# nv-dvl/nerfmatch

Measured on AMD Instinct MI355X. Metric: rays*samples/sec, higher is better.
Workload: dtype fp16x3 (fp16 MFMA on hi/lo-split fp32 operands, three products per fp32 product, fp32 accumulate; fp32 everywhere else)

## Files before the change

### nerfmatch_amd/csrc/nerf_bf16_common.h

```cpp
#pragma once
#include "bf16x3.h"
#include <string.h>

namespace nmbf {

constexpr int TILE = 128;
constexpr int SLOT_BYTES = 16384;
constexpr int SLOT_FLOATS = SLOT_BYTES / 4;
constexpr int NRING = 4;
constexpr int WS_WORKGROUPS = 512;
constexpr int XS = 6;
constexpr int HS = 16;
constexpr int VS = 3;
constexpr int NSLOT_NORGB = XS + 4 * HS + (XS + HS) + 2 * HS;
constexpr int NSLOT_FULL = NSLOT_NORGB + (HS + VS);

constexpr int OFF_BIAS = 0, OFF_BVIEWS = 2304, OFF_WALPHA = 2432, OFF_WRGB = 2688, OFF_MISC = 3072;
constexpr int OFF_SCALE = 3088, OFF_DESCALE = 3104, OFF_INSCALE = 3112, SMALL = 3120;
constexpr int NRANGE = 10;
constexpr int SMALL_PAD = 4096;
constexpr int NSLOT_PAD = 4;
constexpr size_t BLOB_BYTES = (size_t)SMALL_PAD * 4 + (size_t)(NSLOT_FULL + NSLOT_PAD) * SLOT_BYTES;
constexpr int NSLOT_FULL_PAIRED = NSLOT_NORGB + HS / 2 + 2;
constexpr size_t BLOB_BYTES_FP16 = (size_t)SMALL_PAD * 4 + (size_t)(NSLOT_FULL + 8) * (SLOT_BYTES / 2);
constexpr int NSLOT_BWD = 8 + 8 + 16 * 9;
constexpr size_t BLOB_BYTES_BWD = (size_t)SMALL_PAD * 4 + (size_t)(NSLOT_BWD + NSLOT_PAD) * SLOT_BYTES;

constexpr int LDS_SMALL = 0;
constexpr int LDS_RING = SMALL_PAD;
constexpr int LDS_IPE = LDS_RING + NRING * SLOT_FLOATS;
constexpr int LDS_SCR = LDS_IPE + 4 * XS * 2 * 64 * 4;
constexpr int LDS_FEAT = LDS_SCR + TILE * 12 + 32;
constexpr int LDS_EX = LDS_FEAT + 4 * 256;
constexpr int LDS_LEFT = LDS_EX + 4 * 48;
constexpr int LDS_RNG = LDS_LEFT + 2 * TILE;
constexpr int LDS_TOTAL = LDS_RNG + NRANGE * 256;

struct NerfArgs {
  const char* blob;
  const float* rays;
  const float* t;
  const float* app_row;
  float* weights;
  float* feat;
  float* pts;
  float* rgb;
  float* depth;
  float* acc;
  float* raw;
  float* sfeat;
  float* ws;
  int R, S, tap, white_bg, flags, ntiles;
  int Sa;
  int left;
  int ntiles_full;
  const int* tail_viol;
  float var_scale;
  int* status;
};

#ifndef NM_TRACE
#define NM_TRACE 0
#endif

__device__ __forceinline__ int launder(int v) {
  asm volatile("" : "+v"(v));
  return v;
}
__device__ __forceinline__ int launder_s(int v) {
  asm volatile("" : "+s"(v));
  return v;
}

#if NM_TRACE
#define TRACE(i)                                                                                               \
  do {                                                                                                         \
    if (a.raw && threadIdx.x == 0) reinterpret_cast<unsigned long long*>(a.raw)[bid * 32 + (i)] = __builtin_amdgcn_s_memtime(); \
  } while (0)
#else
#define TRACE(i) do { } while (0)
#endif

__device__ __forceinline__ float acc_read(float av) {
  asm volatile("" : "+v"(av));
  return av;
}

template <class T>
__device__ __forceinline__ void pin(T& v) {
  asm volatile("" : "+v"(v));
}
__device__ __forceinline__ float sin32(float x) {
  const float q = __builtin_rintf(x * 0.318309886183790671537767526745028724f);
  float d = __builtin_fmaf(q, -3.140625f, x);
  d = __builtin_fmaf(q, -0.0009670257568359375f, d);
  d = __builtin_fmaf(q, -6.2771141529083251953e-07f, d);
  d = __builtin_fmaf(q, -1.2154201256553420762e-10f, d);
  const float s = d * d;
  d = ((int)q & 1) ? -d : d;
  float u = 2.6083159809786593541503e-06f;
  u = __builtin_fmaf(u, s, -0.0001981069071916863322258f);
  u = __builtin_fmaf(u, s, 0.00833307858556509017944336f);
  u = __builtin_fmaf(u, s, -0.166666597127914428710938f);
  return __builtin_fmaf(s, u * d, d);
}


}
```

### nerfmatch_amd/csrc/nerf_fwd_bf16.hip

```cpp
#include "nerf_split_chain.h"

namespace {
using namespace nmbf;

template <int PART>
__device__ __forceinline__ void tap_prefetch(Ctx& cx) {
  if constexpr (PART == 0) __builtin_amdgcn_s_barrier();
  const char* src = reinterpret_cast<const char*>(cx.tapw);
#pragma unroll
  for (int q = (PART == 0 ? 0 : 4); q < (PART == 0 ? 4 : 7); ++q) {
    const char* sp = src + q * 4096;
    const float* dp = q < 4 ? cx.tap_ring + q * 1024 : cx.tap_ipe + (q - 4) * 1024;
    const unsigned lds = (unsigned)__builtin_amdgcn_readfirstlane((int)(unsigned)(size_t)(const __attribute__((address_space(3))) float*)dp);
    unsigned m0_saved;
    asm volatile("s_mov_b32 %0, m0\n\ts_mov_b32 m0, %1\n\tglobal_load_lds_dwordx4 %2, off\n\tglobal_load_lds_dwordx4 %2, off offset:1024\n\t"
                 "global_load_lds_dwordx4 %2, off offset:2048\n\tglobal_load_lds_dwordx4 %2, off offset:3072\n\ts_mov_b32 m0, %0"
                 : "=&s"(m0_saved) : "s"(lds), "v"(sp) : "memory");
  }
}

__device__ __forceinline__ void dpp_pairs8(float (&o)[8], const float (&x)[8], const float (&y)[8], bool eight) {
  if (eight)
    asm("s_nop 1\n"
        "v_add_f32_dpp %0, %8, %8 row_mirror row_mask:0xf bank_mask:0x3\n\tv_add_f32_dpp %1, %9, %9 row_mirror row_mask:0xf bank_mask:0x3\n\t"
// ... 20 lines not shown
        : "=&v"(o[0]), "=&v"(o[1]), "=&v"(o[2]), "=&v"(o[3]), "=&v"(o[4]), "=&v"(o[5]), "=&v"(o[6]), "=&v"(o[7])
        : "v"(x[0]), "v"(x[1]), "v"(x[2]), "v"(x[3]), "v"(x[4]), "v"(x[5]), "v"(x[6]), "v"(x[7]),
          "v"(y[0]), "v"(y[1]), "v"(y[2]), "v"(y[3]), "v"(y[4]), "v"(y[5]), "v"(y[6]), "v"(y[7]));
}
template <int XOR>
__device__ __forceinline__ void quad_add8(float (&v)[8]) {
  if (XOR == 1)
    asm("s_nop 1\n"
        "v_add_f32_dpp %0, %0, %0 quad_perm:[1,0,3,2] row_mask:0xf bank_mask:0xf\n\tv_add_f32_dpp %1, %1, %1 quad_perm:[1,0,3,2] row_mask:0xf bank_mask:0xf\n\t"
        "v_add_f32_dpp %2, %2, %2 quad_perm:[1,0,3,2] row_mask:0xf bank_mask:0xf\n\tv_add_f32_dpp %3, %3, %3 quad_perm:[1,0,3,2] row_mask:0xf bank_mask:0xf\n\t"
        "v_add_f32_dpp %4, %4, %4 quad_perm:[1,0,3,2] row_mask:0xf bank_mask:0xf\n\tv_add_f32_dpp %5, %5, %5 quad_perm:[1,0,3,2] row_mask:0xf bank_mask:0xf\n\t"
        "v_add_f32_dpp %6, %6, %6 quad_perm:[1,0,3,2] row_mask:0xf bank_mask:0xf\n\tv_add_f32_dpp %7, %7, %7 quad_perm:[1,0,3,2] row_mask:0xf bank_mask:0xf"
        : "+v"(v[0]), "+v"(v[1]), "+v"(v[2]), "+v"(v[3]), "+v"(v[4]), "+v"(v[5]), "+v"(v[6]), "+v"(v[7]));
  else
    asm("s_nop 1\n"
        "v_add_f32_dpp %0, %0, %0 quad_perm:[2,3,0,1] row_mask:0xf bank_mask:0xf\n\tv_add_f32_dpp %1, %1, %1 quad_perm:[2,3,0,1] row_mask:0xf bank_mask:0xf\n\t"
        "v_add_f32_dpp %2, %2, %2 quad_perm:[2,3,0,1] row_mask:0xf bank_mask:0xf\n\tv_add_f32_dpp %3, %3, %3 quad_perm:[2,3,0,1] row_mask:0xf bank_mask:0xf\n\t"
        "v_add_f32_dpp %4, %4, %4 quad_perm:[2,3,0,1] row_mask:0xf bank_mask:0xf\n\tv_add_f32_dpp %5, %5, %5 quad_perm:[2,3,0,1] row_mask:0xf bank_mask:0xf\n\t"
        "v_add_f32_dpp %6, %6, %6 quad_perm:[2,3,0,1] row_mask:0xf bank_mask:0xf\n\tv_add_f32_dpp %7, %7, %7 quad_perm:[2,3,0,1] row_mask:0xf bank_mask:0xf"
        : "+v"(v[0]), "+v"(v[1]), "+v"(v[2]), "+v"(v[3]), "+v"(v[4]), "+v"(v[5]), "+v"(v[6]), "+v"(v[7]));
}
__device__ __forceinline__ float reduce_scatter_step16(float x, float y) {
  const auto r = __builtin_amdgcn_permlane16_swap(__float_as_uint(x), __float_as_uint(y), false, false);
  return __uint_as_float(r[0]) + __uint_as_float(r[1]);
}
__device__ __forceinline__ f32x4 reduce_scatter_16pairs(const float (&s1)[64], int lane) {
  float s2[32];
#pragma unroll
  for (int b = 0; b < 4; ++b) {
    float o[8], x[8], y[8];
#pragma unroll
    for (int i = 0; i < 8; ++i) { x[i] = s1[8 * b + i]; y[i] = s1[32 + 8 * b + i]; }
    dpp_pairs8(o, x, y, true);
#pragma unroll
    for (int i = 0; i < 8; ++i) s2[8 * b + i] = o[i];
  }
  float s3[16];
#pragma unroll
  for (int b = 0; b < 2; ++b) {
    float o[8], x[8], y[8];
#pragma unroll
    for (int i = 0; i < 8; ++i) { x[i] = s2[8 * b + i]; y[i] = s2[16 + 8 * b + i]; }
    dpp_pairs8(o, x, y, false);
#pragma unroll
    for (int i = 0; i < 8; ++i) s3[8 * b + i] = o[i];
  }
  float lo8[8], hi8[8];
#pragma unroll
  for (int i = 0; i < 8; ++i) { lo8[i] = s3[i]; hi8[i] = s3[8 + i]; }
  quad_add8<2>(lo8); quad_add8<2>(hi8);
  float s4[8];
#pragma unroll
  for (int i = 0; i < 8; ++i) s4[i] = (lane & 2) ? hi8[i] : lo8[i];
  float t8[8] = {s4[0], s4[1], s4[2], s4[3], s4[4], s4[5], s4[6], s4[7]};
  quad_add8<1>(t8);
  return (lane & 1) ? f32x4{t8[4], t8[5], t8[6], t8[7]} : f32x4{t8[0], t8[1], t8[2], t8[3]};
}
__device__ __forceinline__ f32x4 reduce_scatter_32rows(float (&v)[128], int lane) {
  float s1[64];
#pragma unroll
  for (int i = 0; i < 64; ++i) s1[i] = reduce_scatter_step16(v[i], v[64 + i]);
  return reduce_scatter_16pairs(s1, lane);
}

#define NM_MLP_DONE_WAIT() __builtin_amdgcn_s_waitcnt(0x0070)
#define NM_EPI_BARRIER() asm volatile("s_waitcnt lgkmcnt(0)\n\ts_barrier" ::: "memory")
template <int P>
__device__ __forceinline__ void nerf_fwd_body(const NerfArgs& a) {
  __shared__ __attribute__((aligned(16))) float sm[LDS_TOTAL];
  float* const sm_small = sm + LDS_SMALL;
  float* const ring = sm + LDS_RING;
  float* const sm_ipe = sm + LDS_IPE;
  float* const sm_sigma = sm + LDS_SCR;
  float* const sm_rgb = sm_sigma + TILE;
  float* const sm_t0 = sm_rgb + 3 * TILE;
  float* const sm_t1 = sm_t0 + TILE;
  float* const sm_mean = sm_t1 + TILE;
  float* const sm_dn = sm_mean + 3 * TILE;
  float* const sm_w = sm_dn + TILE;
  float* const sm_misc = sm_w + TILE;
  float* const sm_part = sm_misc + 32;
  float* const sm_feat = sm + LDS_FEAT;
  float* const sm_ex = sm + LDS_EX;
  int* const sm_lray = reinterpret_cast<int*>(sm + LDS_LEFT);
  float* const sm_lT = sm + LDS_LEFT + TILE;
  unsigned* const sm_rng = reinterpret_cast<unsigned*>(sm + LDS_RNG);

  const int tid = threadIdx.x, lane = tid & 63, wave = tid >> 6, s = lane & 31, hi = lane >> 5;
  const bool tail_ok = a.left && !(a.tail_viol && *a.tail_viol != 0);
  const int S = a.S, R = a.R;
  const int Sa = tail_ok ? a.Sa : S;
  const int left = tail_ok ? 1 : 0;
  const int ntiles = tail_ok ? a.ntiles : a.ntiles_full;
  const int SP = Sa < TILE ? Sa : TILE;
  const int nr = TILE / SP;
  const int nchunks = (Sa + TILE - 1) / TILE;
  const bool need_rgb = !(a.flags & NM_NERF_SKIP_RGB);
  const bool feat_max = (a.flags & NM_NERF_FEAT_MAX) != 0;
  const bool need_tap = (a.feat != nullptr) || (a.sfeat != nullptr);
  const int tap = (a.tap < 0 || a.tap > 7) ? 7 : a.tap;
  const int nslots = need_rgb ? NSLOT_FULL : NSLOT_NORGB;
  const char* const blob_slots = a.blob + (size_t)SMALL_PAD * 4;

  for (int i = tid; i < SMALL / 4; i += 256) reinterpret_cast<f32x4*>(sm_small)[i] = reinterpret_cast<const f32x4*>(a.blob)[i];
  if constexpr (P == 2) {
#pragma unroll
    for (int k = 0; k < NRANGE; ++k) sm_rng[k * 256 + tid] = 0u;
  }

  int nleft = 0;
  int bid = blockIdx.x;
#pragma unroll 1
  for (;;) {
  bool lo_pass = false;
  if (left && (nleft > TILE - 4 || (bid >= ntiles && nleft > 0))) lo_pass = true;
  else if (bid >= ntiles) break;
  const int nent = lo_pass ? nleft : 0;
  TRACE(0);
  if (need_rgb && !lo_pass && tid < nr * 48) {
    const int r2 = tid / 48, f = tid % 48;
    const int ray2 = bid * nr + r2;
    const float* rq = a.rays + (size_t)(ray2 < R ? ray2 : R - 1) * 12 + 8;
    float v = 0.f;
    if (f < 24) {
      const int k = (f % 12) / 3;
      const float xe = rq[f % 3] * (float)(1 << k);
      v = nm_sinf(f < 12 ? xe : xe + 1.57079637050628662109375f);
    } else if (f < 27) {
      v = rq[f - 24];
    } else if (f < 43) {
      v = a.app_row ? a.app_row[f - 27] : 0.f;
    }
    if constexpr (P == 2) {
      v *= reinterpret_cast<const float*>(a.blob)[OFF_INSCALE + (f < 27 ? 1 : 2)];
      __hip_atomic_fetch_max(sm_rng + 9 * 256 + tid, __float_as_uint(fabsf(v)), __ATOMIC_RELAXED, __HIP_MEMORY_SCOPE_WORKGROUP);
    }
    sm_ex[tid] = v;
  }
  __syncthreads();
  TRACE(1);

  const int js = wave * 32 + s;
  const int rl = js / SP;
  const int ray = lo_pass ? (js < nent ? sm_lray[js] : R) : bid * nr + rl;
  const int rc = lo_pass ? sm_lray[js < nent ? js : 0] : (ray < R ? ray : R - 1);
  const float* rp = a.rays + (size_t)rc * 12;
  const float o0 = rp[0], o1 = rp[1], o2 = rp[2], d0 = rp[3], d1 = rp[4], d2 = rp[5], radius = rp[11];
  const float dsq0 = d0 * d0, dsq1 = d1 * d1, dsq2 = d2 * d2;
  const float dmag = fmaxf(1e-10f, (dsq0 + dsq1) + dsq2);
  const float dnorm = sqrtf((dsq0 + dsq1) + dsq2);
  const float nul0 = 1.0f - dsq0 / dmag, nul1 = 1.0f - dsq1 / dmag, nul2 = 1.0f - dsq2 / dmag;

  float red_acc = 0.f;
  float carryT = 1.f;
  float best_w = -1.f;
  float feat_run = 0.f;

  const int nch = lo_pass ? 1 : nchunks;
  for (int chunk = 0; chunk < nch; ++chunk) {
    const int sidx = lo_pass ? Sa : chunk * TILE + (js % SP);
    const float t0 = a.t[(size_t)rc * (S + 1) + sidx];
    const float t1 = a.t[(size_t)rc * (S + 1) + sidx + 1];
    const float mu = (t0 + t1) / 2.0f, hw = (t1 - t0) / 2.0f;
    const float mu2 = mu * mu, hw2 = hw * hw, hw4 = hw2 * hw2;
    const float denom = fmaxf(1.1920928955078125e-07f, 3.0f * mu2 + hw2);
    const float t_mean = mu + (2.0f * mu * hw2) / denom;
    const float t_var = hw2 / 3.0f - (float)(4.0 / 15.0) * ((hw4 * (12.0f * mu2 - hw2)) / (denom * denom));
    const float r_var = (radius * radius) * ((mu2 / 4.0f + (float)(5.0 / 12.0) * hw2) - (float)(4.0 / 15.0) * hw4 / denom);
    float mean[3] = {d0 * t_mean + o0, d1 * t_mean + o1, d2 * t_mean + o2};
    float var[3] = {t_var * dsq0 + r_var * nul0, t_var * dsq1 + r_var * nul1, t_var * dsq2 + r_var * nul2};
    if (a.var_scale > 0.f) {
      var[0] *= a.var_scale; var[1] *= a.var_scale; var[2] *= a.var_scale;
    }
    if (hi == 0) {
      sm_t0[js] = t0; sm_t1[js] = t1;
      sm_mean[js] = mean[0]; sm_mean[TILE + js] = mean[1]; sm_mean[2 * TILE + js] = mean[2];
      sm_dn[js] = dnorm;
    }

#pragma unroll
    for (int g0 = 0; g0 < ring_ahead<P>(); ++g0) dma_slot<P>(blob_slots, g0, ring, wave, lane);

    {
      float* dst = sm_ipe + wave * (XS * 2 * 64 * 4) + lane * 4;
      const float ipe_scale = sm_small[OFF_INSCALE];
      const float phl = hi ? 1.57079637050628662109375f : 0.f;
#pragma unroll
      for (int m = 0; m < XS; ++m) {
        float v8[8];
#pragma unroll
        for (int i = 0; i < 8; ++i) {
          const int idx = 8 * m + i;
          const bool live = idx < 45;
          const int ax = (live ? idx : 0) % 3, sb = (live ? idx : 0) / 3;
          const float mu = mean[ax], vr = var[ax];
          const float sc = (float)(1 << sb);
          const float xe = mu * sc;
          float v = __builtin_amdgcn_exp2f((-0.5f * (vr * (sc * sc))) * 1.44269504088896340736f) * sin32(xe + phl);
          if constexpr (P == 2) v *= ipe_scale;
          v8[i] = live ? v : 0.f;
        }
        if constexpr (is_split<P>()) {
          bf16x8 h8, l8;
          split8_p<P>(v8, h8, l8);
          *reinterpret_cast<u32x4*>(dst + (m * 2 + 0) * 256) = __builtin_bit_cast(u32x4, h8);
          *reinterpret_cast<u32x4*>(dst + (m * 2 + 1) * 256) = __builtin_bit_cast(u32x4, l8);
        } else {
          *reinterpret_cast<u32x4*>(dst + m * 256) = __builtin_bit_cast(u32x4, pack8_f16(v8));
        }
      }
    }

    TRACE(2);
    Ctx cx;
    cx.blob_slots = blob_slots; cx.ring = ring; cx.sm_small = sm_small;
    cx.tapw = reinterpret_cast<f32x4*>(a.ws) + ((size_t)blockIdx.x * 4 + wave) * 32 * 64 + lane;
    cx.nslots = nslots; cx.wave = wave; cx.lane = lane; cx.hi = hi; cx.tap = need_tap ? tap : -1; cx.g = 0; cx.sig_part = 0.f;
    cx.vmax = 0.f; cx.rng = sm_rng + tid; cx.sc = 1.f;
    const bool early = need_rgb && !lo_pass && tap == 7 && a.feat && !a.sfeat;
    cx.tap_pref = need_tap && !lo_pass && !early; cx.rgb = need_rgb;
// ... 54 lines not shown
          if (a.raw && !NM_TRACE) {
            f32x4 rv = {sm_rgb[tid2], sm_rgb[TILE + tid2], sm_rgb[2 * TILE + tid2], sm_sigma[tid2]};
            *reinterpret_cast<f32x4*>(a.raw + ((size_t)ray2 * S + s2) * 4) = rv;
          }
        }
        float pq[8] = {wgt, wgt * sm_rgb[tid2], wgt * sm_rgb[TILE + tid2], wgt * sm_rgb[2 * TILE + tid2],
                       wgt * (0.5f * (sm_t0[tid2] + sm_t1[tid2])), wgt * sm_mean[tid2], wgt * sm_mean[TILE + tid2],
                       wgt * sm_mean[2 * TILE + tid2]};
        nm_half_sum_dpp8(pq);
        if ((tid2 & 31) == 16) {
          *reinterpret_cast<f32x4*>(sm_part + (tid2 >> 5) * 8) = f32x4{pq[0], pq[1], pq[2], pq[3]};
          *reinterpret_cast<f32x4*>(sm_part + (tid2 >> 5) * 8 + 4) = f32x4{pq[4], pq[5], pq[6], pq[7]};
        }
      }
    };
    auto pick_best = [&]() __attribute__((always_inline)) {
      const int tid2 = launder(threadIdx.x);
      if (tid2 < 8 * nr) {
        const int q = tid2 & 7, r2 = tid2 >> 3;
        const float* wv = sm_w + r2 * SP;
        float bw = wv[0];
        int bi = 0;
        for (int k = 1; k < SP; ++k)
          if (wv[k] > bw) { bw = wv[k]; bi = k; }
        const bool better = bw > best_w;
        if (better) best_w = bw;
        if (q == 0) sm_misc[8 + r2] = better ? __int_as_float(r2 * SP + bi) : __int_as_float(-1);
        if (q >= 5 && better) red_acc = sm_mean[(q - 5) * TILE + r2 * SP + bi];
      }
    };
    auto tap7_early = [&](Ctx& c) __attribute__((always_inline)) {
      const int t2 = launder(threadIdx.x), jl = (t2 >> 6) * 32 + (t2 & 31), hl = (t2 >> 5) & 1;
      const float sigma_raw = (c.sig_part + nm_shfl_xor32(c.sig_part)) + sm_small[OFF_MISC];
      if (hl == 0) sm_sigma[jl] = sigma_raw;
      NM_EPI_BARRIER();
      composite_weights();
      NM_EPI_BARRIER();
      if (feat_max) {
        pick_best();
        NM_EPI_BARRIER();
      }
      const float desc = sm_small[OFF_DESCALE + 7];
      const float wj = sm_w[jl] * desc;
      const int best = feat_max ? __float_as_int(sm_misc[8 + jl / SP]) : -2;
      const float mult = feat_max ? (jl == best ? desc : 0.f) : wj;
      const float* bl = sm_small + OFF_BIAS + 7 * 256 + 4 * hl;
      const float s7 = sm_small[OFF_SCALE + 7];
      float s1[64];
#pragma unroll
      for (int cq = 0; cq < HS; ++cq) {
        const f32x4 b0 = *reinterpret_cast<const f32x4*>(bl + (cq >> 2) * 32 + 8 * (cq & 3));
        const f32x4 b1 = *reinterpret_cast<const f32x4*>(bl + (4 + (cq >> 2)) * 32 + 8 * (cq & 3));
#pragma unroll
        for (int e = 0; e < 4; ++e) {
          const float x = mult * __builtin_fmaxf(__builtin_fmaf(c.hv[4 * cq + e], s7, b0[e]), 0.f);
          const float y = mult * __builtin_fmaxf(__builtin_fmaf(c.hv[64 + 4 * cq + e], s7, b1[e]), 0.f);
          s1[4 * cq + e] = reduce_scatter_step16(x, y);
        }
      }
      const f32x4 sum4 = reduce_scatter_16pairs(s1, jl);
      const int r = jl & 31;
      float* prow = sm_feat + (jl >> 5) * 256 + 4 * hl;
      *reinterpret_cast<f32x4*>(prow + (r >> 2) * 32 + 16 * ((r >> 1) & 1) + 8 * (r & 1)) = sum4;
    };
    const Tap7InRegisters<decltype(tap7_early)> tap7{early, tap7_early};
    f32x16 acc[8];
    ipe_steps<P, true>(acc, cx, ipe_src);
    finish_layer<P>(acc, 0, cx);
    TRACE(3);
#pragma unroll 1
    for (int l = 1; l < 8; ++l) {
      layer_pass<P>(acc, l, cx, ipe_src, tap7);
      TRACE(3 + l);
    }
    float c_r = 0.f, c_g = 0.f, c_b = 0.f;
    if (!need_rgb) {
      if (cx.tap == 7) dump_tap(7, cx);
      NM_MLP_DONE_WAIT();
      if (cx.tap_pref) tap_prefetch<0>(cx);
      alpha_head(cx);
      if (cx.tap_pref) tap_prefetch<1>(cx);
    } else {
      const int hh = launder(lane) >> 5;
      const float* exr = sm_ex + launder(rl) * 48 + 8 * hh;
      f32x16 av[4];
      views_hidden<P>(av, cx);
      fold_range<P>(cx, 7);
      bf16x8 exh[VS], exl[VS];
#pragma unroll
      for (int e = 0; e < VS; ++e) {
        float v8[8];
        if (!lo_pass) {
          const f32x4 e0 = *reinterpret_cast<const f32x4*>(exr + 16 * e), e1 = *reinterpret_cast<const f32x4*>(exr + 16 * e + 4);
          v8[0] = e0[0]; v8[1] = e0[1]; v8[2] = e0[2]; v8[3] = e0[3]; v8[4] = e1[0]; v8[5] = e1[1]; v8[6] = e1[2]; v8[7] = e1[3];
        } else {
          const float* rq = a.rays + (size_t)launder(rc) * 12 + 8;
          const float vd0 = rq[0], vd1 = rq[1], vd2 = rq[2];
#pragma unroll
          for (int i = 0; i < 8; ++i) {
            const int f = 16 * e + 8 * hh + i;
            const int ax = f % 3;
            const float dax = ax == 0 ? vd0 : ax == 1 ? vd1 : vd2;
            float v = 0.f;
            if (f < 24) {
              const float xe = dax * (float)(1 << ((f % 12) / 3));
              v = nm_sinf(f < 12 ? xe : xe + 1.57079637050628662109375f);
            } else if (f < 27) {
              v = dax;
            } else if (f < 43) {
              v = a.app_row ? a.app_row[f - 27] : 0.f;
            }
            if constexpr (P == 2) v *= sm_small[OFF_INSCALE + (f < 27 ? 1 : 2)];
            v8[i] = v;
          }
        }
        if constexpr (is_split<P>()) split8_p<P>(v8, exh[e], exl[e]);
        else exh[e] = exl[e] = pack8_f16(v8);
      }
      views_extras<P>(av, cx, exh, exl);
      TRACE(11);
      NM_MLP_DONE_WAIT();
      if (cx.tap_pref) tap_prefetch<0>(cx);
      const float* bv = sm_small + OFF_BVIEWS + 4 * hh;
      const float* wr = sm_small + OFF_WRGB + 4 * hh;
      float pr = 0.f, pg = 0.f, pb = 0.f;
#pragma unroll
      for (int ob = 0; ob < 4; ++ob) {
#pragma unroll
        for (int q = 0; q < 4; ++q) {
          const f32x4 b4 = *reinterpret_cast<const f32x4*>(bv + ob * 32 + 8 * q);
          const f32x4 wr4 = *reinterpret_cast<const f32x4*>(wr + ob * 32 + 8 * q);
          const f32x4 wg4 = *reinterpret_cast<const f32x4*>(wr + 128 + ob * 32 + 8 * q);
          const f32x4 wb4 = *reinterpret_cast<const f32x4*>(wr + 256 + ob * 32 + 8 * q);
#pragma unroll
          for (int e = 0; e < 4; ++e) {
            const float hv = __builtin_fmaxf(acc_read(av[ob][4 * q + e]) + b4[e], 0.f);
            pr = NM_FMA(hv, wr4[e], pr);
            pg = NM_FMA(hv, wg4[e], pg);
            pb = NM_FMA(hv, wb4[e], pb);
          }
        }
      }
      pr = (pr + nm_shfl_xor32(pr)) + sm_small[OFF_MISC + 1];
      pg = (pg + nm_shfl_xor32(pg)) + sm_small[OFF_MISC + 2];
      pb = (pb + nm_shfl_xor32(pb)) + sm_small[OFF_MISC + 3];
      c_r = 1.0f / (1.0f + expf(-pr));
      c_g = 1.0f / (1.0f + expf(-pg));
      c_b = 1.0f / (1.0f + expf(-pb));
      if (cx.tap_pref) tap_prefetch<1>(cx);
    }
    const float sigma_raw = (cx.sig_part + nm_shfl_xor32(cx.sig_part)) + sm_small[OFF_MISC];
    TRACE(12);
    {
      const int jsw = launder(js);
      if ((launder(lane) >> 5) == 0) {
        sm_sigma[jsw] = sigma_raw;
        sm_rgb[jsw] = c_r; sm_rgb[TILE + jsw] = c_g; sm_rgb[2 * TILE + jsw] = c_b;
      }
    }
    NM_EPI_BARRIER();
    TRACE(13);
    const int tid2 = launder(threadIdx.x), lane2 = tid2 & 63, wave2 = tid2 >> 6;

    if (lo_pass) {
      if (tid2 < nent) {
        const int ray2 = sm_lray[tid2];
        const float sg = fmaxf(sm_sigma[tid2], 0.f);
        const float delta = (sm_t1[tid2] - sm_t0[tid2]) * sm_dn[tid2];
        const float wgt = (1.0f - expf(-sg * delta)) * sm_lT[tid2];
        sm_w[tid2] = wgt;
        a.weights[(size_t)ray2 * S + Sa] = wgt;
        if (a.acc) atomicAdd(a.acc + ray2, wgt);
        if (a.rgb && need_rgb) {
#pragma unroll
          for (int c = 0; c < 3; ++c) atomicAdd(a.rgb + (size_t)ray2 * 3 + c, a.white_bg ? wgt * sm_rgb[c * TILE + tid2] - wgt : wgt * sm_rgb[c * TILE + tid2]);
        }
        if (a.depth) atomicAdd(a.depth + ray2, wgt * (0.5f * (sm_t0[tid2] + sm_t1[tid2])));
        if (a.pts) {
#pragma unroll
          for (int c = 0; c < 3; ++c) atomicAdd(a.pts + (size_t)ray2 * 3 + c, wgt * sm_mean[c * TILE + tid2]);
        }
      }
      __syncthreads();
      if (need_tap) {
        const int jl = launder(js), hl = launder(lane) >> 5;
        const f32x4* tw = reinterpret_cast<const f32x4*>(a.ws) + ((size_t)blockIdx.x * 4 + wave2) * 32 * 64 + lane2;
        if (jl < nent) {
          const int ray2 = sm_lray[jl];
          const float desc = sm_small[OFF_DESCALE + tap];
          const float wj = sm_w[jl] * desc;
#pragma unroll 4
          for (int ks = 0; ks < HS; ++ks) {
            const f32x4 ta = tw[(2 * ks) * 64], tb = tw[(2 * ks + 1) * 64];
            const int n0 = (ks >> 1) * 32 + 16 * (ks & 1) + 4 * hl;
            if (a.sfeat) {
              float* dsf = a.sfeat + ((size_t)ray2 * S + Sa) * 256 + n0;
              *reinterpret_cast<f32x4*>(dsf) = ta * desc;
              *reinterpret_cast<f32x4*>(dsf + 8) = tb * desc;
            }
            if (a.feat) {
              float* df = a.feat + (size_t)ray2 * 256 + n0;
#pragma unroll
              for (int e = 0; e < 4; ++e) {
                atomicAdd(df + e, wj * ta[e]);
                atomicAdd(df + 8 + e, wj * tb[e]);
              }
            }
          }
        }
      }
      __syncthreads();
      break;
    }

    if (!early) composite_weights();
    composite_sums();
    NM_EPI_BARRIER();

    if (tid2 < 8 * nr) {
// ... 173 lines not shown
```

### nerfmatch_amd/csrc/nerf_pack_bf16.hip

```cpp
#include "nerf_bf16_common.h"
#include <stdlib.h>

namespace {
using namespace nmbf;

inline uint16_t bf16_rne(float f) {
  uint32_t u;
  memcpy(&u, &f, 4);
  if ((u & 0x7fffffffu) > 0x7f800000u) return (uint16_t)((u >> 16) | 0x40);
  u += 0x7fffu + ((u >> 16) & 1u);
  return (uint16_t)(u >> 16);
}
inline float bf16_to_f(uint16_t h) {
  uint32_t u = (uint32_t)h << 16;
  float f;
  memcpy(&f, &u, 4);
  return f;
}

inline uint16_t f16_bits(float f) {
  f = f > 65504.0f ? 65504.0f : (f < -65504.0f ? -65504.0f : f);
  const _Float16 hf = (_Float16)f;
  uint16_t bits;
  memcpy(&bits, &hf, 2);
// ... 83 lines not shown
    for (int k = 0; k < 256; ++k) {
      double acc = 0.0;
      for (int j = 0; j < 256; ++j) acc += (double)vr[j] * (double)w->feat_w[(size_t)j * 256 + k];
      fv.W[(size_t)n * ldv + k] = (float)acc;
    }
    for (int c = 256; c < ldv; ++c) fv.W[(size_t)n * ldv + c] = vr[c];
    double bb = (double)w->views_b[n];
    for (int j = 0; j < 256; ++j) bb += (double)vr[j] * (double)w->feat_b[j];
    fv.b[n] = (float)bb;
  }
  return NM_OK;
}

static int choose_fp16_scales(const nmNerfWeights* w, const float* views_folded, const int* act_log2, Fp16Scales& sc) {
  sc.c[0] = 12; sc.c[10] = 12; sc.c[11] = 0;
  if (act_log2) {
    for (int i = 0; i < 12; ++i) {
      if (act_log2[i] < -24 || act_log2[i] > 15) return NM_ERR_ARG;
      sc.c[i] = act_log2[i];
    }
    if (sc.c[0] > 15 || sc.c[10] > 15) return NM_ERR_ARG;
  }
  const int ldv = 283 + w->app_dim;
  sc.a0 = weight_exp(absmax_cols(w->pts_w[0], 256, 90, 0, 90));
  sc.A[0] = sc.a0 + sc.c[0];
  for (int l = 1; l < 8; ++l) {
    const float* W = w->pts_w[l];
    const int ld = l == 5 ? 346 : 256, col0 = l == 5 ? 90 : 0;
    sc.ah[l] = weight_exp(absmax_cols(W, 256, ld, col0, col0 + 256));
    sc.A[l] = sc.ah[l] + sc.c[l];
  }
  {
    const int ideal = weight_exp(absmax_cols(w->pts_w[5], 256, 346, 0, 90));
    sc.ax5 = sc.A[5] - sc.c[0];
    if (sc.ax5 > ideal + 1) {
      const int d = sc.ax5 - (ideal + 1);
      sc.ax5 -= d; sc.ah[5] -= d; sc.A[5] -= d;
    }
  }
  {
    sc.c[9] = sc.c[8];
    sc.ah[9] = weight_exp(absmax_cols(views_folded, 128, ldv, 0, 256));
    sc.A[9] = sc.ah[9] + sc.c[9];
    const int ideal_d = weight_exp(absmax_cols(views_folded, 128, ldv, 256, 283));
    const int ideal_a = w->app_dim ? weight_exp(absmax_cols(views_folded, 128, ldv, 283, ldv)) : 1 << 20;
    int d = 0;
    if (sc.A[9] - sc.c[10] > ideal_d + 1) d = sc.A[9] - sc.c[10] - (ideal_d + 1);
    if (sc.A[9] - sc.c[11] - d > ideal_a + 1) d = sc.A[9] - sc.c[11] - (ideal_a + 1);
    sc.ah[9] -= d; sc.A[9] -= d;
    sc.avd = sc.A[9] - sc.c[10];
    sc.ava = sc.A[9] - sc.c[11];
  }
  for (int i = 0; i < 10; ++i)
    if (sc.A[i] < -100 || sc.A[i] > 100) return NM_ERR_ARG;
  return NM_OK;
}

static int nerf_pack_split(const nmNerfWeights* w, void* blob_v, int fp16, const int* act_log2 = nullptr) {
  if (!w || !blob_v) return NM_ERR_ARG;
  for (int i = 0; i < 8; ++i)
    if (!w->pts_w[i] || !w->pts_b[i]) return NM_ERR_ARG;
  if (!w->alpha_w || !w->alpha_b || !w->feat_w || !w->feat_b || !w->views_w || !w->views_b || !w->rgb_w || !w->rgb_b)
    return NM_ERR_ARG;
  if (w->app_dim != 0 && w->app_dim != 16) return NM_ERR_UNSUPPORTED;
  FoldedViews fv;
  if (fold_views(w, fv) != NM_OK) return NM_ERR_ARG;
  Fp16Scales sc;
  if (fp16 == 2) {
    const int rc = choose_fp16_scales(w, fv.W, act_log2, sc);
    if (rc != NM_OK) return rc;
  }
  auto p2 = [](int e) { return ldexpf(1.0f, e); };
  memset(blob_v, 0, fp16 == 1 ? BLOB_BYTES_FP16 : BLOB_BYTES);
  float* small = (float*)blob_v;
  for (int l = 0; l < 8; ++l)
    for (int n = 0; n < 256; ++n) small[OFF_BIAS + l * 256 + n] = w->pts_b[l][n] * p2(sc.c[l + 1]);
  for (int n = 0; n < 128; ++n) small[OFF_BVIEWS + n] = fv.b[n] * p2(sc.A[9]);
  for (int n = 0; n < 256; ++n) small[OFF_WALPHA + n] = w->alpha_w[n] * p2(-sc.c[8]);
  for (int n = 0; n < 384; ++n) small[OFF_WRGB + n] = w->rgb_w[n] * p2(-sc.A[9]);
  small[OFF_MISC] = w->alpha_b[0];
  for (int c = 0; c < 3; ++c) small[OFF_MISC + 1 + c] = w->rgb_b[c];
  for (int l = 0; l < 16; ++l) small[OFF_SCALE + l] = l < 8 ? p2(sc.c[l + 1] - sc.A[l]) : 1.0f;
  for (int l = 0; l < 8; ++l) small[OFF_DESCALE + l] = p2(-sc.c[l + 1]);
  small[OFF_INSCALE + 0] = p2(sc.c[0]); small[OFF_INSCALE + 1] = p2(sc.c[10]); small[OFF_INSCALE + 2] = p2(sc.c[11]); small[OFF_INSCALE + 3] = 1.0f;

  uint16_t* slots = (uint16_t*)((char*)blob_v + (size_t)SMALL_PAD * 4);
  int g = 0;
  auto next = [&]() { return slots + (size_t)(g++) * ((fp16 == 1 ? SLOT_BYTES / 2 : SLOT_BYTES) / 2); };
  auto ipe_steps = [&](const float* W, int ld, int aexp) {
    const float f = p2(aexp);
    for (int m = 0; m < XS; ++m)
      pack_slot(next(), W, ld, 8, [&](int h, int i) { const int idx = 8 * m + i; return idx < 45 ? 45 * h + idx : -1; }, fp16, [&](int) { return f; });
  };
  auto hid_steps = [&](const float* W, int ld, int col0, int nob, int aexp) {
    const float f = p2(aexp);
    for (int ks = 0; ks < HS; ++ks)
      pack_slot(next(), W, ld, nob, [&](int h, int i) { return col0 + 32 * (ks >> 1) + nrow(8 * (ks & 1) + i, h); }, fp16, [&](int) { return f; });
  };
  for (int l = 0; l < 8; ++l) {
    if (l == 0) ipe_steps(w->pts_w[0], 90, sc.a0);
    if (l != 0) hid_steps(w->pts_w[l], l == 5 ? 346 : 256, l == 5 ? 90 : 0, 8, sc.ah[l]);
    if (l == 5) ipe_steps(w->pts_w[5], 346, sc.ax5);
  }
  const int ldv = 283 + w->app_dim;
  const float fvh = p2(sc.ah[9]), fvd = p2(sc.avd), fva = p2(sc.ava);
  auto hid_col = [&](int ks, int h, int i) { return 32 * (ks >> 1) + nrow(8 * (ks & 1) + i, h); };
  auto ext_col = [&](int e, int h, int i) {
    const int f = 16 * e + 8 * h + i;
    if (f < 27) return 256 + f;
    if (f < 43 && w->app_dim) return 283 + (f - 27);
    return -1;
  };
  auto vsc = [&](int c) { return c < 256 ? fvh : c < 283 ? fvd : fva; };
  if (fp16 != 1) {
    for (int sl = 0; sl < HS / 2; ++sl)
      pack_slot2(next(), fv.W, ldv, [&](int h, int i) { return hid_col(2 * sl, h, i); }, [&](int h, int i) { return hid_col(2 * sl + 1, h, i); }, fp16, vsc);
    pack_slot2(next(), fv.W, ldv, [&](int h, int i) { return ext_col(0, h, i); }, [&](int h, int i) { return ext_col(1, h, i); }, fp16, vsc);
    pack_slot(next(), fv.W, ldv, 4, [&](int h, int i) { return ext_col(2, h, i); }, fp16, vsc);
    return g == NSLOT_FULL_PAIRED ? NM_OK : NM_ERR_ARG;
  }
  hid_steps(fv.W, ldv, 0, 4, sc.ah[9]);
  for (int e = 0; e < VS; ++e) pack_slot(next(), fv.W, ldv, 4, [&](int h, int i) { return ext_col(e, h, i); }, fp16, vsc);
  return g == NSLOT_FULL ? NM_OK : NM_ERR_ARG;
}

extern "C" int nm_nerf_pack_bf16x3(const nmNerfWeights* w, void* blob_v) { return nerf_pack_split(w, blob_v, 0); }
extern "C" int nm_nerf_pack_fp16x3(const nmNerfWeights* w, const int* act_log2, void* blob_v) { return nerf_pack_split(w, blob_v, 2, act_log2); }
extern "C" int nm_nerf_pack_fp16x1(const nmNerfWeights* w, void* blob_v) { return nerf_pack_split(w, blob_v, 1); }

extern "C" int nm_nerf_pack_bwd_bf16x3(const nmNerfWeights* w, void* blob_v) {
  if (!w || !blob_v) return NM_ERR_ARG;
  void* tmp = malloc(BLOB_BYTES);
  if (!tmp) return NM_ERR_ARG;
  const int rc = nerf_pack_split(w, tmp, 0);
  if (rc != NM_OK) { free(tmp); return rc; }
  memset(blob_v, 0, BLOB_BYTES_BWD);
  memcpy(blob_v, tmp, (size_t)SMALL_PAD * 4);
  free(tmp);
  uint16_t* slots = (uint16_t*)((char*)blob_v + (size_t)SMALL_PAD * 4);
  int g = 0;
  auto next = [&]() { return slots + (size_t)(g++) * (SLOT_BYTES / 2); };
  const int ldv = 283 + w->app_dim;
  auto product = [&](int n_out, int n_in, int nob, auto wt) {
    float* T = (float*)calloc((size_t)32 * nob * n_in, sizeof(float));
    for (int o = 0; o < n_out; ++o)
      for (int k = 0; k < n_in; ++k) T[(size_t)o * n_in + k] = wt(o, k);
    for (int ks = 0; ks < n_in / 16; ++ks)
      pack_slot(next(), T, n_in, nob, [&](int h, int i) { return 32 * (ks >> 1) + nrow(8 * (ks & 1) + i, h); }, 0, [](int) { return 1.0f; });
    free(T);
  };
  const int nxd = 27 + w->app_dim;
  FoldedViews fv;
  if (fold_views(w, fv) != NM_OK) return NM_ERR_ARG;
  product(nxd, 128, 4, [&](int c, int n) { return w->views_w[(size_t)n * ldv + 256 + c]; });
  product(256, 128, 8, [&](int k, int n) { return fv.W[(size_t)n * ldv + k]; });
  for (int l = 7; l >= 6; --l) product(256, 256, 8, [&](int k, int n) { return w->pts_w[l][(size_t)n * 256 + k]; });
  product(90, 256, 4, [&](int f, int n) { return w->pts_w[5][(size_t)n * 346 + f]; });
  product(256, 256, 8, [&](int k, int n) { return w->pts_w[5][(size_t)n * 346 + 90 + k]; });
  for (int l = 4; l >= 1; --l) product(256, 256, 8, [&](int k, int n) { return w->pts_w[l][(size_t)n * 256 + k]; });
  product(90, 256, 4, [&](int f, int n) { return w->pts_w[0][(size_t)n * 90 + f]; });
  return g == NSLOT_BWD ? NM_OK : NM_ERR_ARG;
}
```

### nerfmatch_amd/csrc/nerf_split_chain.h

```cpp
#pragma once
#include "nerf_bf16_common.h"

namespace nmbf {

template <int P> constexpr bool is_bf16() { return P == 0 || P == 4; }
template <int P> constexpr bool has_gates() { return P == 4; }
typedef _Float16 f16x8 __attribute__((ext_vector_type(8)));
typedef _Float16 f16x2 __attribute__((ext_vector_type(2)));
template <int P>
__device__ __forceinline__ f32x16 mfma_p(const bf16x8& a, const bf16x8& b, const f32x16& c) {
  if constexpr (is_bf16<P>()) return MFMA_BF16(a, b, c);
  else return __builtin_amdgcn_mfma_f32_32x32x16_f16(__builtin_bit_cast(f16x8, a), __builtin_bit_cast(f16x8, b), c, 0, 0, 0);
}
template <int P> constexpr bool is_split() { return P != 1; }
template <int P> constexpr int slot_bytes() { return is_split<P>() ? SLOT_BYTES : SLOT_BYTES / 2; }
template <int P> constexpr int slot_floats() { return slot_bytes<P>() / 4; }
template <int P> constexpr int ring_slots() { return is_split<P>() ? NRING : 2 * NRING; }
template <int P> constexpr int ring_ahead() { return is_split<P>() ? 4 : 6; }
constexpr float F16_MAX = 65504.0f;
__device__ __forceinline__ void split8_f16(const float (&v)[8], bf16x8& hi, bf16x8& lo) {
  f16x8 h8, l8;
#pragma unroll
  for (int i = 0; i < 8; ++i) {
    const float c = __builtin_amdgcn_fmed3f(v[i], -F16_MAX, F16_MAX);
// ... 394 lines not shown
    acc[o] = mfma_p<P>(C.h[o], xh, FIRST ? zero : acc[o]);
    __builtin_amdgcn_sched_barrier(0);
    work(o);
    __builtin_amdgcn_sched_barrier(0);
  }
  load_half<P>(cx.opA, cx.ring + ((g + 1) & (NRING - 1)) * SLOT_FLOATS, cx.lane, 0);
  __builtin_amdgcn_sched_barrier(0);
#pragma unroll
  for (int o = 0; o < 4; ++o) {
    acc[o] = mfma_p<P>(C.h[o], xl, acc[o]);
    __builtin_amdgcn_sched_barrier(0);
    work(4 + o);
    __builtin_amdgcn_sched_barrier(0);
  }
#pragma unroll
  for (int o = 0; o < 4; ++o) {
    acc[o] = mfma_p<P>(C.l[o], xh, acc[o]);
    __builtin_amdgcn_sched_barrier(0);
    work(8 + o);
    __builtin_amdgcn_sched_barrier(0);
  }
  cx.g = g + 1;
}

template <int P, bool FIRST, bool EVEN, class W0, class W1>
__device__ __forceinline__ void slot_step4x2(f32x16 (&av)[4], Ctx& cx, const bf16x8& x0h, const bf16x8& x0l, Unit& u1, W0 w0, W1 w1) {
  const f32x16 zero = {0.f, 0.f, 0.f, 0.f, 0.f, 0.f, 0.f, 0.f, 0.f, 0.f, 0.f, 0.f, 0.f, 0.f, 0.f, 0.f};
  const int g = cx.g;
  const OpHalf A = cx.opA;
  OpHalf B;
  w0.prefetch();
#pragma unroll
  for (int o = 0; o < 4; ++o) {
    av[o] = mfma_p<P>(A.h[o], x0h, FIRST ? zero : av[o]);
    __builtin_amdgcn_sched_barrier(0);
    w0(o);
    __builtin_amdgcn_sched_barrier(0);
  }
  load_half<P>(B, cx.ring + (g & (NRING - 1)) * SLOT_FLOATS, cx.lane, 1);
  __builtin_amdgcn_sched_barrier(0);
#pragma unroll
  for (int o = 0; o < 4; ++o) {
    av[o] = mfma_p<P>(A.h[o], x0l, av[o]);
    __builtin_amdgcn_sched_barrier(0);
    w0(4 + o);
    __builtin_amdgcn_sched_barrier(0);
  }
#pragma unroll
  for (int o = 0; o < 4; ++o) {
    av[o] = mfma_p<P>(A.l[o], x0h, av[o]);
    __builtin_amdgcn_sched_barrier(0);
    w0(8 + o);
    __builtin_amdgcn_sched_barrier(0);
  }
  if constexpr (!EVEN) ring_acquire_two<P>(cx.blob_slots, g, cx.ring, cx.wave, cx.lane);
  const bf16x8 x1h = __builtin_bit_cast(bf16x8, u1.h), x1l = __builtin_bit_cast(bf16x8, u1.l);
  w1.prefetch();
#pragma unroll
  for (int o = 0; o < 4; ++o) {
    av[o] = mfma_p<P>(B.h[o], x1h, av[o]);
    __builtin_amdgcn_sched_barrier(0);
    w1(o);
    __builtin_amdgcn_sched_barrier(0);
  }
  load_half<P>(cx.opA, cx.ring + ((g + 1) & (NRING - 1)) * SLOT_FLOATS, cx.lane, 0);
  __builtin_amdgcn_sched_barrier(0);
#pragma unroll
  for (int o = 0; o < 4; ++o) {
    av[o] = mfma_p<P>(B.h[o], x1l, av[o]);
    __builtin_amdgcn_sched_barrier(0);
    w1(4 + o);
    __builtin_amdgcn_sched_barrier(0);
  }
#pragma unroll
  for (int o = 0; o < 4; ++o) {
    av[o] = mfma_p<P>(B.l[o], x1h, av[o]);
    __builtin_amdgcn_sched_barrier(0);
    w1(8 + o);
    __builtin_amdgcn_sched_barrier(0);
  }
  cx.g = g + 1;
}

template <int P>
__device__ __forceinline__ void views_hidden(f32x16 (&av)[4], Ctx& cx) {
  if constexpr (is_split<P>()) {
#pragma unroll
    for (int sl = 0; sl < HS / 2; ++sl) {
      const Unit x0 = cx.xn;
      Unit u1;
      const bf16x8 x0h = __builtin_bit_cast(bf16x8, x0.h), x0l = __builtin_bit_cast(bf16x8, x0.l);
      if (sl == 0) slot_step4x2<P, true, true>(av, cx, x0h, x0l, u1, unit_work<P>(1, 7, cx, u1), unit_work<P>(2, 7, cx, cx.xn));
      else if (sl + 1 == HS / 2) slot_step4x2<P, false, false>(av, cx, x0h, x0l, u1, unit_work<P>(2 * sl + 1, 7, cx, u1), NoWork{});
      else if (sl & 1) slot_step4x2<P, false, false>(av, cx, x0h, x0l, u1, unit_work<P>(2 * sl + 1, 7, cx, u1), unit_work<P>(2 * sl + 2, 7, cx, cx.xn));
      else slot_step4x2<P, false, true>(av, cx, x0h, x0l, u1, unit_work<P>(2 * sl + 1, 7, cx, u1), unit_work<P>(2 * sl + 2, 7, cx, cx.xn));
    }
  } else {
#pragma unroll
    for (int ks = 0; ks < HS; ks += 2) {
      {
        const Unit xc = cx.xn;
        if (ks == 0) slot_step4<P, true, true>(av, cx, __builtin_bit_cast(bf16x8, xc.h), __builtin_bit_cast(bf16x8, xc.l), unit_work<P>(ks + 1, 7, cx, cx.xn));
        else slot_step4<P, false, true>(av, cx, __builtin_bit_cast(bf16x8, xc.h), __builtin_bit_cast(bf16x8, xc.l), unit_work<P>(ks + 1, 7, cx, cx.xn));
      }
      {
        const Unit xc = cx.xn;
        if (ks + 2 < HS) slot_step4<P, false, false>(av, cx, __builtin_bit_cast(bf16x8, xc.h), __builtin_bit_cast(bf16x8, xc.l), unit_work<P>(ks + 2, 7, cx, cx.xn));
        else slot_step4<P, false, false>(av, cx, __builtin_bit_cast(bf16x8, xc.h), __builtin_bit_cast(bf16x8, xc.l), NoWork{});
      }
    }
  }
}
template <int P>
__device__ __forceinline__ void views_extras(f32x16 (&av)[4], Ctx& cx, const bf16x8 (&eh)[VS], const bf16x8 (&el)[VS]) {
  if constexpr (is_split<P>()) {
    Unit u1;
    u1.h = __builtin_bit_cast(u32x4, eh[1]); u1.l = __builtin_bit_cast(u32x4, el[1]);
    slot_step4x2<P, false, true>(av, cx, eh[0], el[0], u1, NoWork{}, NoWork{});
    slot_step4<P, false, false>(av, cx, eh[2], el[2], NoWork{});
  } else {
#pragma unroll
    for (int e = 0; e < VS; ++e) {
      if (e & 1) slot_step4<P, false, false>(av, cx, eh[e], el[e], NoWork{});
      else slot_step4<P, false, true>(av, cx, eh[e], el[e], NoWork{});
    }
  }
}

template <int P, bool FIRST>
__device__ __forceinline__ void ipe_steps(f32x16 (&acc)[8], Ctx& cx, const float* ipe_src) {
  auto operand = [&](int m, bf16x8& ph, bf16x8& pl) {
    ph = __builtin_bit_cast(bf16x8, *reinterpret_cast<const u32x4*>(ipe_src + (is_split<P>() ? (m * 2 + 0) : m) * 256));
    pl = ph;
    if constexpr (is_split<P>()) pl = __builtin_bit_cast(bf16x8, *reinterpret_cast<const u32x4*>(ipe_src + (m * 2 + 1) * 256));
  };
#pragma unroll
  for (int m = 0; m < XS; m += 2) {
    bf16x8 ph, pl;
    operand(m, ph, pl);
    if (m == 0) slot_step8<P, FIRST, true>(acc, cx, ph, pl, NoWork{});
    else slot_step8<P, false, true>(acc, cx, ph, pl, NoWork{});
    operand(m + 1, ph, pl);
    if (m + 2 == XS) slot_step8<P, false, false>(acc, cx, ph, pl, AccTake<P>{acc, cx});
    else slot_step8<P, false, false>(acc, cx, ph, pl, NoWork{});
  }
}

struct Tap7Workspace {
  static constexpr bool on = false;
  __device__ __forceinline__ void fn(Ctx&) const {}
};
template <class F>
struct Tap7InRegisters {
  bool on;
  F fn;
};

template <int P, class Tap7 = Tap7Workspace>
__device__ __forceinline__ void layer_pass(f32x16 (&acc)[8], int l, Ctx& cx, const float* ipe_src, const Tap7& tap7 = Tap7()) {
  if (l - 1 == cx.tap) dump_tap(l - 1, cx);
#pragma unroll
  for (int ks = 0; ks < HS; ks += 2) {
    {
      const Unit xc = cx.xn;
      if (ks == 0) slot_step8<P, true, true>(acc, cx, __builtin_bit_cast(bf16x8, xc.h), __builtin_bit_cast(bf16x8, xc.l), unit_work<P>(ks + 1, l - 1, cx, cx.xn));
      else slot_step8<P, false, true>(acc, cx, __builtin_bit_cast(bf16x8, xc.h), __builtin_bit_cast(bf16x8, xc.l), unit_work<P>(ks + 1, l - 1, cx, cx.xn));
    }
    {
      const Unit xc = cx.xn;
      if (ks + 2 < HS) slot_step8<P, false, false>(acc, cx, __builtin_bit_cast(bf16x8, xc.h), __builtin_bit_cast(bf16x8, xc.l), unit_work<P>(ks + 2, l - 1, cx, cx.xn));
      else slot_step8<P, false, false>(acc, cx, __builtin_bit_cast(bf16x8, xc.h), __builtin_bit_cast(bf16x8, xc.l), AccTake<P>{acc, cx});
    }
  }
  fold_range<P>(cx, l - 1);
  if constexpr (has_gates<P>()) {
    cx.gptr[(l - 1) * 256] = u32x4{cx.gbits[0], cx.gbits[1], cx.gbits[2], cx.gbits[3]};
    cx.gbits[0] = cx.gbits[1] = cx.gbits[2] = cx.gbits[3] = 0u;
  }
  if (l == 5) ipe_steps<P, false>(acc, cx, ipe_src);
  finish_layer<P>(acc, l, cx);
  if (l == 7) {
    if (cx.rgb) {
      if (cx.tap == 7 && !tap7.on) dump_tap(7, cx);
      alpha_head(cx);
      if (tap7.on) tap7.fn(cx);
// ... 6 lines not shown
```

Baseline: 367.7 million.

## Precompute per-ray view-layer contribution once per tile instead of per-sample MFMA

The view-dependent layer's input (view-direction encoding plus appearance code) is constant along a ray, so its product with the weight columns is now computed once per ray at tile start, in fp32 FMAs against a repacked weight section in the blob. The result (bias folded in) seeds the MFMA accumulators, and the per-sample extras MFMA slots (views_extras) are skipped for normal tiles. This removes three MFMA slot steps and their split/pack work per sample. In exchange it adds a barrier and extra per-ray prologue work and a new blob section, and the leftover-ray path keeps the old route.

```diff
diff --git a/nerfmatch_amd/csrc/nerf_bf16_common.h b/nerfmatch_amd/csrc/nerf_bf16_common.h
--- a/nerfmatch_amd/csrc/nerf_bf16_common.h
+++ b/nerfmatch_amd/csrc/nerf_bf16_common.h
@@ -22,7 +22,12 @@
 constexpr int NSLOT_PAD = 4;
 constexpr size_t BLOB_BYTES = (size_t)SMALL_PAD * 4 + (size_t)(NSLOT_FULL + NSLOT_PAD) * SLOT_BYTES;
 constexpr int NSLOT_FULL_PAIRED = NSLOT_NORGB + HS / 2 + 2;
-constexpr size_t BLOB_BYTES_FP16 = (size_t)SMALL_PAD * 4 + (size_t)(NSLOT_FULL + 8) * (SLOT_BYTES / 2);
+constexpr int RAYTERM_ROWS = 44, RAYTERM_FLOATS = RAYTERM_ROWS * 128;
+constexpr int NSLOT_RENDER_PAIRED = NSLOT_NORGB + HS / 2;
+constexpr size_t RAYTERM_OFF = (size_t)SMALL_PAD * 4 + (size_t)(NSLOT_FULL_PAIRED + NSLOT_PAD + 2) * SLOT_BYTES;
+static_assert(RAYTERM_OFF + (size_t)RAYTERM_FLOATS * 4 <= BLOB_BYTES, "the per-ray section must fit behind the paired slots");
+constexpr size_t RAYTERM_OFF_FP16 = (size_t)SMALL_PAD * 4 + (size_t)(NSLOT_FULL + 8) * (SLOT_BYTES / 2);
+constexpr size_t BLOB_BYTES_FP16 = RAYTERM_OFF_FP16 + (size_t)RAYTERM_FLOATS * 4;
 constexpr int NSLOT_BWD = 8 + 8 + 16 * 9;
 constexpr size_t BLOB_BYTES_BWD = (size_t)SMALL_PAD * 4 + (size_t)(NSLOT_BWD + NSLOT_PAD) * SLOT_BYTES;
 
@@ -32,7 +37,8 @@
 constexpr int LDS_SCR = LDS_IPE + 4 * XS * 2 * 64 * 4;
 constexpr int LDS_FEAT = LDS_SCR + TILE * 12 + 32;
 constexpr int LDS_EX = LDS_FEAT + 4 * 256;
-constexpr int LDS_LEFT = LDS_EX + 4 * 48;
+constexpr int LDS_URAY = LDS_EX + 4 * 48;
+constexpr int LDS_LEFT = LDS_URAY + 4 * 128;
 constexpr int LDS_RNG = LDS_LEFT + 2 * TILE;
 constexpr int LDS_TOTAL = LDS_RNG + NRANGE * 256;
 
diff --git a/nerfmatch_amd/csrc/nerf_fwd_bf16.hip b/nerfmatch_amd/csrc/nerf_fwd_bf16.hip
--- a/nerfmatch_amd/csrc/nerf_fwd_bf16.hip
+++ b/nerfmatch_amd/csrc/nerf_fwd_bf16.hip
@@ -126,6 +126,7 @@
   float* const sm_part = sm_misc + 32;
   float* const sm_feat = sm + LDS_FEAT;
   float* const sm_ex = sm + LDS_EX;
+  float* const sm_u = sm + LDS_URAY;
   int* const sm_lray = reinterpret_cast<int*>(sm + LDS_LEFT);
   float* const sm_lT = sm + LDS_LEFT + TILE;
   unsigned* const sm_rng = reinterpret_cast<unsigned*>(sm + LDS_RNG);
@@ -145,6 +146,7 @@
   const int tap = (a.tap < 0 || a.tap > 7) ? 7 : a.tap;
   const int nslots = need_rgb ? NSLOT_FULL : NSLOT_NORGB;
   const char* const blob_slots = a.blob + (size_t)SMALL_PAD * 4;
+  const float* const rayterm = reinterpret_cast<const float*>(a.blob + (is_split<P>() ? RAYTERM_OFF : RAYTERM_OFF_FP16));
 
   for (int i = tid; i < SMALL / 4; i += 256) reinterpret_cast<f32x4*>(sm_small)[i] = reinterpret_cast<const f32x4*>(a.blob)[i];
   if constexpr (P == 2) {
@@ -161,25 +163,53 @@
   else if (bid >= ntiles) break;
   const int nent = lo_pass ? nleft : 0;
   TRACE(0);
-  if (need_rgb && !lo_pass && tid < nr * 48) {
-    const int r2 = tid / 48, f = tid % 48;
-    const int ray2 = bid * nr + r2;
-    const float* rq = a.rays + (size_t)(ray2 < R ? ray2 : R - 1) * 12 + 8;
-    float v = 0.f;
-    if (f < 24) {
-      const int k = (f % 12) / 3;
-      const float xe = rq[f % 3] * (float)(1 << k);
-      v = nm_sinf(f < 12 ? xe : xe + 1.57079637050628662109375f);
-    } else if (f < 27) {
-      v = rq[f - 24];
-    } else if (f < 43) {
-      v = a.app_row ? a.app_row[f - 27] : 0.f;
-    }
-    if constexpr (P == 2) {
-      v *= reinterpret_cast<const float*>(a.blob)[OFF_INSCALE + (f < 27 ? 1 : 2)];
-      __hip_atomic_fetch_max(sm_rng + 9 * 256 + tid, __float_as_uint(fabsf(v)), __ATOMIC_RELAXED, __HIP_MEMORY_SCOPE_WORKGROUP);
-    }
-    sm_ex[tid] = v;
+  if (need_rgb && !lo_pass) {
+    const int t2 = launder(threadIdx.x), n = t2 & 127, r0 = t2 >> 7;
+    const float* const rt_col = rayterm + n;
+    float vd[27];
+#pragma unroll
+    for (int k = 0; k < 27; ++k) vd[k] = rt_col[k * 128];
+    const float vbias = rt_col[43 * 128];
+    const float units = reinterpret_cast<const float*>(a.blob)[launder_s(OFF_INSCALE + 3)];
+    if (t2 < nr * 48) {
+      const int r2 = t2 / 48, f = t2 % 48;
+      const int ray2 = bid * nr + r2;
+      const float* rq = a.rays + (size_t)(ray2 < R ? ray2 : R - 1) * 12 + 8;
+      float v = 0.f;
+      if (f < 24) {
+        const int k = (f % 12) / 3;
+        const float xe = rq[f % 3] * (float)(1 << k);
+        v = nm_sinf(f < 12 ? xe : xe + 1.57079637050628662109375f);
+      } else if (f < 27) {
+        v = rq[f - 24];
+      } else if (f < 43) {
+        v = a.app_row ? a.app_row[f - 27] : 0.f;
+      }
+      if constexpr (P == 2) {
+        const float vs = v * reinterpret_cast<const float*>(a.blob)[OFF_INSCALE + (f < 27 ? 1 : 2)];
+        __hip_atomic_fetch_max(sm_rng + 9 * 256 + t2, __float_as_uint(fabsf(vs)), __ATOMIC_RELAXED, __HIP_MEMORY_SCOPE_WORKGROUP);
+      }
+      sm_ex[t2] = v;
+    }
+    NM_EPI_BARRIER();
+    const float* e0 = sm_ex + r0 * 48;
+    const float* e1 = sm_ex + (r0 + 2) * 48;
+    float u0 = vbias, u1 = vbias;
+#pragma unroll
+    for (int k = 0; k < 27; ++k) {
+      u0 = __builtin_fmaf(vd[k], e0[k], u0);
+      u1 = __builtin_fmaf(vd[k], e1[k], u1);
+    }
+    if (a.app_row) {
+#pragma unroll
+      for (int k = 0; k < 16; ++k) {
+        const float va = rt_col[(27 + k) * 128];
+        u0 = __builtin_fmaf(va, e0[27 + k], u0);
+        u1 = __builtin_fmaf(va, e1[27 + k], u1);
+      }
+    }
+    if (r0 < nr) sm_u[r0 * 128 + n] = u0 * units;
+    if (r0 + 2 < nr) sm_u[(r0 + 2) * 128 + n] = u1 * units;
   }
   __syncthreads();
   TRACE(1);
@@ -400,20 +430,16 @@
       if (cx.tap_pref) tap_prefetch<1>(cx);
     } else {
       const int hh = launder(lane) >> 5;
-      const float* exr = sm_ex + launder(rl) * 48 + 8 * hh;
       f32x16 av[4];
-      views_hidden<P>(av, cx);
+      views_hidden<P, true>(av, cx, (lo_pass ? sm_small + OFF_BVIEWS : sm_u + launder(rl) * 128) + 4 * hh);
       fold_range<P>(cx, 7);
-      bf16x8 exh[VS], exl[VS];
-#pragma unroll
-      for (int e = 0; e < VS; ++e) {
-        float v8[8];
-        if (!lo_pass) {
-          const f32x4 e0 = *reinterpret_cast<const f32x4*>(exr + 16 * e), e1 = *reinterpret_cast<const f32x4*>(exr + 16 * e + 4);
-          v8[0] = e0[0]; v8[1] = e0[1]; v8[2] = e0[2]; v8[3] = e0[3]; v8[4] = e1[0]; v8[5] = e1[1]; v8[6] = e1[2]; v8[7] = e1[3];
-        } else {
-          const float* rq = a.rays + (size_t)launder(rc) * 12 + 8;
-          const float vd0 = rq[0], vd1 = rq[1], vd2 = rq[2];
+      if (lo_pass) {
+        bf16x8 exh[VS], exl[VS];
+        const float* rq = a.rays + (size_t)launder(rc) * 12 + 8;
+        const float vd0 = rq[0], vd1 = rq[1], vd2 = rq[2];
+#pragma unroll
+        for (int e = 0; e < VS; ++e) {
+          float v8[8];
 #pragma unroll
           for (int i = 0; i < 8; ++i) {
             const int f = 16 * e + 8 * hh + i;
@@ -431,28 +457,26 @@
             if constexpr (P == 2) v *= sm_small[OFF_INSCALE + (f < 27 ? 1 : 2)];
             v8[i] = v;
           }
-        }
-        if constexpr (is_split<P>()) split8_p<P>(v8, exh[e], exl[e]);
-        else exh[e] = exl[e] = pack8_f16(v8);
-      }
-      views_extras<P>(av, cx, exh, exl);
+          if constexpr (is_split<P>()) split8_p<P>(v8, exh[e], exl[e]);
+          else exh[e] = exl[e] = pack8_f16(v8);
+        }
+        views_extras<P>(av, cx, exh, exl);
+      }
       TRACE(11);
       NM_MLP_DONE_WAIT();
       if (cx.tap_pref) tap_prefetch<0>(cx);
-      const float* bv = sm_small + OFF_BVIEWS + 4 * hh;
       const float* wr = sm_small + OFF_WRGB + 4 * hh;
       float pr = 0.f, pg = 0.f, pb = 0.f;
 #pragma unroll
       for (int ob = 0; ob < 4; ++ob) {
 #pragma unroll
         for (int q = 0; q < 4; ++q) {
-          const f32x4 b4 = *reinterpret_cast<const f32x4*>(bv + ob * 32 + 8 * q);
           const f32x4 wr4 = *reinterpret_cast<const f32x4*>(wr + ob * 32 + 8 * q);
           const f32x4 wg4 = *reinterpret_cast<const f32x4*>(wr + 128 + ob * 32 + 8 * q);
           const f32x4 wb4 = *reinterpret_cast<const f32x4*>(wr + 256 + ob * 32 + 8 * q);
 #pragma unroll
           for (int e = 0; e < 4; ++e) {
-            const float hv = __builtin_fmaxf(acc_read(av[ob][4 * q + e]) + b4[e], 0.f);
+            const float hv = __builtin_fmaxf(acc_read(av[ob][4 * q + e]), 0.f);
             pr = NM_FMA(hv, wr4[e], pr);
             pg = NM_FMA(hv, wg4[e], pg);
             pb = NM_FMA(hv, wb4[e], pb);
diff --git a/nerfmatch_amd/csrc/nerf_pack_bf16.hip b/nerfmatch_amd/csrc/nerf_pack_bf16.hip
--- a/nerfmatch_amd/csrc/nerf_pack_bf16.hip
+++ b/nerfmatch_amd/csrc/nerf_pack_bf16.hip
@@ -189,7 +189,16 @@
   for (int c = 0; c < 3; ++c) small[OFF_MISC + 1 + c] = w->rgb_b[c];
   for (int l = 0; l < 16; ++l) small[OFF_SCALE + l] = l < 8 ? p2(sc.c[l + 1] - sc.A[l]) : 1.0f;
   for (int l = 0; l < 8; ++l) small[OFF_DESCALE + l] = p2(-sc.c[l + 1]);
-  small[OFF_INSCALE + 0] = p2(sc.c[0]); small[OFF_INSCALE + 1] = p2(sc.c[10]); small[OFF_INSCALE + 2] = p2(sc.c[11]); small[OFF_INSCALE + 3] = 1.0f;
+  small[OFF_INSCALE + 0] = p2(sc.c[0]); small[OFF_INSCALE + 1] = p2(sc.c[10]); small[OFF_INSCALE + 2] = p2(sc.c[11]); small[OFF_INSCALE + 3] = p2(sc.A[9]);
+  {
+    float* rt = (float*)((char*)blob_v + (fp16 == 1 ? RAYTERM_OFF_FP16 : RAYTERM_OFF));
+    const int ldw = 283 + w->app_dim;
+    for (int n = 0; n < 128; ++n) {
+      for (int k = 0; k < 27; ++k) rt[k * 128 + n] = fv.W[(size_t)n * ldw + 256 + k];
+      for (int k = 0; k < 16; ++k) rt[(27 + k) * 128 + n] = w->app_dim ? fv.W[(size_t)n * ldw + 283 + k] : 0.f;
+      rt[43 * 128 + n] = fv.b[n];
+    }
+  }
 
   uint16_t* slots = (uint16_t*)((char*)blob_v + (size_t)SMALL_PAD * 4);
   int g = 0;
diff --git a/nerfmatch_amd/csrc/nerf_split_chain.h b/nerfmatch_amd/csrc/nerf_split_chain.h
--- a/nerfmatch_amd/csrc/nerf_split_chain.h
+++ b/nerfmatch_amd/csrc/nerf_split_chain.h
@@ -500,15 +500,25 @@
   cx.g = g + 1;
 }
 
-template <int P>
-__device__ __forceinline__ void views_hidden(f32x16 (&av)[4], Ctx& cx) {
+template <int P, bool START = false>
+__device__ __forceinline__ void views_hidden(f32x16 (&av)[4], Ctx& cx, const float* start = nullptr) {
+  if constexpr (START) {
+#pragma unroll
+    for (int ob = 0; ob < 4; ++ob)
+#pragma unroll
+      for (int q = 0; q < 4; ++q) {
+        const f32x4 u4 = *reinterpret_cast<const f32x4*>(start + ob * 32 + 8 * q);
+#pragma unroll
+        for (int e = 0; e < 4; ++e) av[ob][4 * q + e] = u4[e];
+      }
+  }
   if constexpr (is_split<P>()) {
 #pragma unroll
     for (int sl = 0; sl < HS / 2; ++sl) {
       const Unit x0 = cx.xn;
       Unit u1;
       const bf16x8 x0h = __builtin_bit_cast(bf16x8, x0.h), x0l = __builtin_bit_cast(bf16x8, x0.l);
-      if (sl == 0) slot_step4x2<P, true, true>(av, cx, x0h, x0l, u1, unit_work<P>(1, 7, cx, u1), unit_work<P>(2, 7, cx, cx.xn));
+      if (sl == 0) slot_step4x2<P, !START, true>(av, cx, x0h, x0l, u1, unit_work<P>(1, 7, cx, u1), unit_work<P>(2, 7, cx, cx.xn));
       else if (sl + 1 == HS / 2) slot_step4x2<P, false, false>(av, cx, x0h, x0l, u1, unit_work<P>(2 * sl + 1, 7, cx, u1), NoWork{});
       else if (sl & 1) slot_step4x2<P, false, false>(av, cx, x0h, x0l, u1, unit_work<P>(2 * sl + 1, 7, cx, u1), unit_work<P>(2 * sl + 2, 7, cx, cx.xn));
       else slot_step4x2<P, false, true>(av, cx, x0h, x0l, u1, unit_work<P>(2 * sl + 1, 7, cx, u1), unit_work<P>(2 * sl + 2, 7, cx, cx.xn));
@@ -518,7 +528,7 @@
     for (int ks = 0; ks < HS; ks += 2) {
       {
         const Unit xc = cx.xn;
-        if (ks == 0) slot_step4<P, true, true>(av, cx, __builtin_bit_cast(bf16x8, xc.h), __builtin_bit_cast(bf16x8, xc.l), unit_work<P>(ks + 1, 7, cx, cx.xn));
+        if (ks == 0) slot_step4<P, !START, true>(av, cx, __builtin_bit_cast(bf16x8, xc.h), __builtin_bit_cast(bf16x8, xc.l), unit_work<P>(ks + 1, 7, cx, cx.xn));
         else slot_step4<P, false, true>(av, cx, __builtin_bit_cast(bf16x8, xc.h), __builtin_bit_cast(bf16x8, xc.l), unit_work<P>(ks + 1, 7, cx, cx.xn));
       }
       {
```

Result: no change. 374.6 million, median of 6 (+1.9%).
